# PaddlePaddle/PaddleRec

Hardware: AMD Instinct MI355X
Metric: CTR samples/sec, Criteo DeepFM bs=65536 (train step: fwd+bwd+optimizer) (higher is better)
Workload: dtype f32 (MLP GEMMs: f32 operands as 3 bf16 terms, 6 bf16 MFMAs per product, f32 accumulate); 1 GPU; DeepFM full Criteo: 26 sparse slots x 1000000 rows x dim 16, 13 dense, MLP 400,400,400, batch 65536 per GPU, lazy Adam, uniform ids; global_batch=65536, parallelism=single, table_rows_total=26000000, index_oob_flag=0

## Files before the change

### paddlerec_amd/csrc/crossnet_layers.hip

```cpp
#include "rec_common.h"

namespace rec {

__global__ __launch_bounds__(kBlock) void add_into_kernel(int64_t n, float* __restrict__ dst,
                                                          const float* __restrict__ src, int accumulate) {
  for (int64_t i = (int64_t)blockIdx.x * kBlock + threadIdx.x; i < n; i += (int64_t)gridDim.x * kBlock)
    dst[i] = accumulate ? dst[i] + src[i] : src[i];
}

static void add_into(int64_t n, float* dst, const float* src, int accumulate, hipStream_t st) {
  int64_t grid = (n + kBlock - 1) / kBlock;
  if (grid > kNumCU * 8) grid = kNumCU * 8;
  hipLaunchKernelGGL(add_into_kernel, dim3((unsigned)grid), dim3(kBlock), 0, st, n, dst, src, accumulate);
}

struct Carve {
  char* base;
  size_t off = 0;
  explicit Carve(void* p) : base((char*)p) {}
  float* take(size_t floats) {
    float* r = base ? (float*)(base + off) : nullptr;
    off += align_up(floats * sizeof(float), 256);
    return r;
  }
};

static rec_gemm_desc gd(int64_t m, int n, int k, int lda, int ldb, int ldc, int ta, int tb, int epi) {
  rec_gemm_desc d;
  d.m = m; d.n = n; d.k = k; d.lda = lda; d.ldb = ldb; d.ldc = ldc;
  d.trans_a = ta; d.trans_b = tb; d.epilogue = epi; d.split_k = 0;
  return d;
}

static size_t gemm_ws(const rec_gemm_desc& d) {
  size_t b = 0;
  rec_gemm_f32_workspace_bytes(&d, &b);
  return align_up(b, 256);
}

static size_t max2(size_t a, size_t b) { return a > b ? a : b; }

}

using namespace rec;

#define REC_TRY(call)        \
  do {                       \
    if (int rc_ = (call)) return rc_; \
  } while (0)

static int v2_check(const rec_crossnet_v2_desc* d) {
  REC_REQUIRE(d, REC_EINVAL, "desc is NULL");
  REC_REQUIRE(d->batch >= 0 && d->d > 0, REC_EINVAL, "bad sizes B=%lld d=%d", (long long)d->batch, d->d);
  return REC_OK;
}
static int ldx(int ld, int d) { return ld > 0 ? ld : d; }
static int v2_ldmax(const rec_crossnet_v2_desc* d) {
  int m = d->d;
  for (int v : {d->ld_x0, d->ld_xl, d->ld_out, d->ld_u}) m = v > m ? v : m;
  return m;
}
static int mix_ldmax(const rec_crossnet_mix_desc* d) {
  int m = d->d;
  for (int v : {d->ld_x0, d->ld_xl, d->ld_out}) m = v > m ? v : m;
  return m;
}

extern "C" int rec_crossnet_v2_layer_workspace_bytes(const rec_crossnet_v2_desc* d, size_t* fwd_bytes,
                                                     size_t* bwd_bytes) {
  REC_TRY(v2_check(d));
  const int n = d->d;
  const int lw = v2_ldmax(d);
  if (fwd_bytes) *fwd_bytes = gemm_ws(gd(d->batch, n, n, lw, n, lw, 0, 0, REC_EPI_CROSS));
  if (bwd_bytes) {
    const size_t g = max2(gemm_ws(gd(n, n, (int)d->batch, lw, n, n, 1, 0, REC_EPI_NONE)),
                          gemm_ws(gd(d->batch, n, n, n, n, lw, 0, 1, REC_EPI_ADD)));
    *bwd_bytes = align_up((size_t)d->batch * n * sizeof(float), 256) + g;
  }
  return REC_OK;
}

extern "C" int rec_crossnet_v2_layer_fwd(const rec_crossnet_v2_desc* d, const float* X0, const float* Xl,
                                         const float* W, const float* bias, float* Xnext, float* U_saved,
                                         void* workspace, size_t workspace_bytes, void* stream) {
  REC_TRY(v2_check(d));
  if (d->batch == 0) return REC_OK;
  REC_REQUIRE(X0 && Xl && W && bias && Xnext, REC_EINVAL, "null pointer argument");
  const int n = d->d;
  const rec_gemm_desc g = gd(d->batch, n, n, ldx(d->ld_xl, n), n, ldx(d->ld_out, n), 0, 0, REC_EPI_CROSS);
  rec_gemm_epilogue_args a = {};
  a.bias = bias;
  a.aux0 = X0; a.ld_aux0 = ldx(d->ld_x0, n);
  a.aux1 = Xl; a.ld_aux1 = ldx(d->ld_xl, n);
  a.out2 = U_saved; a.ld_out2 = ldx(d->ld_u, n);
  return rec_gemm_f32(&g, Xl, W, Xnext, &a, workspace, workspace_bytes, stream);
}

extern "C" int rec_crossnet_v2_layer_bwd(const rec_crossnet_v2_desc* d, const float* X0, const float* Xl,
                                         const float* W, const float* U_saved, const float* dXnext,
                                         int32_t ld_dxnext, float* dX0_acc, int32_t ld_acc,
                                         int32_t accumulate_dx0, int32_t fold_dx0, float* dXl, int32_t ld_dxl,
                                         float* dW, float* db, void* workspace, size_t workspace_bytes,
                                         void* stream) {
  REC_TRY(v2_check(d));
  if (d->batch == 0) return REC_OK;
  REC_REQUIRE(X0 && Xl && W && U_saved && dXnext && dX0_acc && dXl && dW && db, REC_EINVAL,
              "null pointer argument");
  const int n = d->d;
  size_t need = 0;
  rec_crossnet_v2_layer_workspace_bytes(d, nullptr, &need);
  REC_REQUIRE(workspace && workspace_bytes >= need, REC_EWORKSPACE, "workspace %zu < %zu", workspace_bytes, need);
  Carve c(workspace);
  float* dU = c.take((size_t)d->batch * n);
  void* gws = (char*)workspace + c.off;
  const size_t gws_bytes = workspace_bytes - c.off;
  REC_TRY(rec_cross_bwd_prep(d->batch, n, dXnext, ldx(ld_dxnext, n), X0, ldx(d->ld_x0, n), U_saved,
                             ldx(d->ld_u, n), dU, n, dX0_acc, ldx(ld_acc, n), accumulate_dx0, stream));
  {
    const rec_gemm_desc g = gd(n, n, (int)d->batch, ldx(d->ld_xl, n), n, n, 1, 0, REC_EPI_NONE);
    rec_gemm_epilogue_args a = {};
    a.b_colsum = db;
    REC_TRY(rec_gemm_f32(&g, Xl, dU, dW, &a, gws, gws_bytes, stream));
  }
  {
    const rec_gemm_desc g = gd(d->batch, n, n, n, n, ldx(ld_dxl, n), 0, 1, REC_EPI_ADD);
    rec_gemm_epilogue_args a = {};
    a.aux1 = dXnext; a.ld_aux1 = ldx(ld_dxnext, n);
    if (fold_dx0) { a.aux0 = dX0_acc; a.ld_aux0 = ldx(ld_acc, n); }
    REC_TRY(rec_gemm_f32(&g, dU, W, dXl, &a, gws, gws_bytes, stream));
  }
  return REC_OK;
}

static int mix_check(const rec_crossnet_mix_desc* d) {
  REC_REQUIRE(d, REC_EINVAL, "desc is NULL");
  REC_REQUIRE(d->batch >= 0 && d->d > 0 && d->rank > 0 && d->experts > 0 && d->experts <= 64, REC_EINVAL,
              "bad sizes B=%lld d=%d r=%d E=%d", (long long)d->batch, d->d, d->rank, d->experts);
  return REC_OK;
}

static size_t mix_gemm_ws(const rec_crossnet_mix_desc* d) {
  const int n = d->d, r = d->rank, E = d->experts;
  const int64_t B = d->batch;
  const int lw = mix_ldmax(d);
  size_t g = 0;
  g = max2(g, gemm_ws(gd(B, E, n, lw, E, E, 0, 0, REC_EPI_BIAS)));
  g = max2(g, gemm_ws(gd(B, r, n, lw, r, E * r, 0, 0, REC_EPI_BIAS_TANH)));
  g = max2(g, gemm_ws(gd(B, r, r, E * r, r, E * r, 0, 1, REC_EPI_BIAS_TANH)));
  g = max2(g, gemm_ws(gd(B, n, r, E * r, r, lw, 0, 1, REC_EPI_MOE)));
  g = max2(g, gemm_ws(gd(n, r, (int)B, lw, E * r, r, 1, 0, REC_EPI_NONE)));
  g = max2(g, gemm_ws(gd(r, r, (int)B, r, E * r, r, 1, 0, REC_EPI_NONE)));
  g = max2(g, gemm_ws(gd(B, r, n, n, r, r, 0, 0, REC_EPI_DTANH)));
  g = max2(g, gemm_ws(gd(B, r, r, r, r, r, 0, 0, REC_EPI_DTANH)));
  g = max2(g, gemm_ws(gd(B, n, r, r, r, lw, 0, 1, REC_EPI_ADD)));
  g = max2(g, gemm_ws(gd(n, E, (int)B, lw, E, E, 1, 0, REC_EPI_NONE)));
  g = max2(g, gemm_ws(gd(B, n, E, E, E, lw, 0, 1, REC_EPI_ADD)));
  size_t cs = 0;
  rec_colsum_workspace_bytes(B, n, &cs);
  return max2(g, align_up(cs, 256));
}

extern "C" int rec_crossnet_mix_layer_workspace_bytes(const rec_crossnet_mix_desc* d, size_t* fwd_bytes,
                                                      size_t* bwd_bytes) {
  REC_TRY(mix_check(d));
  const size_t B = (size_t)d->batch, n = d->d, r = d->rank, E = d->experts;
  const size_t g = mix_gemm_ws(d);
  auto al = [](size_t floats) { return align_up(floats * sizeof(float), 256); };
  if (fwd_bytes) *fwd_bytes = al(B * E) + g;
  if (bwd_bytes)
    *bwd_bytes = 2 * al(B * n) + al(B * E) + 2 * al(B * r) + al(B * E) + al(n) + al(n * E) + al(E) + g;
  return REC_OK;
}

extern "C" int rec_crossnet_mix_layer_fwd(const rec_crossnet_mix_desc* d, const float* X0, const float* Xl,
                                          const float* U, const float* V, const float* Cm, const float* bias,
                                          const float* gate_w, const float* gate_b, float* Xnext, float* t1,
                                          float* t2, float* prob, void* workspace, size_t workspace_bytes,
                                          void* stream) {
  REC_TRY(mix_check(d));
  if (d->batch == 0) return REC_OK;
  REC_REQUIRE(X0 && Xl && U && V && Cm && bias && gate_w && gate_b && Xnext && t1 && t2 && prob, REC_EINVAL,
              "null pointer argument");
  const int n = d->d, r = d->rank, E = d->experts;
  const int64_t B = d->batch;
  const int lx0 = ldx(d->ld_x0, n), lxl = ldx(d->ld_xl, n), lo = ldx(d->ld_out, n);
  size_t need = 0;
  rec_crossnet_mix_layer_workspace_bytes(d, &need, nullptr);
  REC_REQUIRE(workspace && workspace_bytes >= need, REC_EWORKSPACE, "workspace %zu < %zu", workspace_bytes, need);
  Carve c(workspace);
  float* gate = c.take((size_t)B * E);
  void* gws = (char*)workspace + c.off;
  const size_t gwb = workspace_bytes - c.off;
  {
    const rec_gemm_desc g = gd(B, E, n, lxl, E, E, 0, 0, REC_EPI_BIAS);
    rec_gemm_epilogue_args a = {};
    a.bias = gate_b;
    REC_TRY(rec_gemm_f32(&g, Xl, gate_w, gate, &a, gws, gwb, stream));
  }
  REC_TRY(rec_softmax_rows(B, E, gate, E, prob, E, stream));
  for (int e = 0; e < E; ++e) {
    {
      const rec_gemm_desc g = gd(B, r, n, lxl, r, E * r, 0, 0, REC_EPI_BIAS_TANH);
      rec_gemm_epilogue_args a = {};
      REC_TRY(rec_gemm_f32(&g, Xl, V + (size_t)e * n * r, t1 + e * r, &a, gws, gwb, stream));
    }
    {
      const rec_gemm_desc g = gd(B, r, r, E * r, r, E * r, 0, 1, REC_EPI_BIAS_TANH);
      rec_gemm_epilogue_args a = {};
      REC_TRY(rec_gemm_f32(&g, t1 + e * r, Cm + (size_t)e * r * r, t2 + e * r, &a, gws, gwb, stream));
    }
  }
  for (int e = 0; e < E; ++e) {
    const rec_gemm_desc g = gd(B, n, r, E * r, r, lo, 0, 1, REC_EPI_MOE);
    rec_gemm_epilogue_args a = {};
    a.bias = bias;
    a.aux0 = X0; a.ld_aux0 = lx0;
    a.aux1 = e == 0 ? Xl : Xnext; a.ld_aux1 = e == 0 ? lxl : lo;
    a.row_scale = prob + e; a.row_scale_stride = E;
    REC_TRY(rec_gemm_f32(&g, t2 + e * r, U + (size_t)e * n * r, Xnext, &a, gws, gwb, stream));
  }
  return REC_OK;
}

extern "C" int rec_crossnet_mix_layer_bwd(const rec_crossnet_mix_desc* d, const float* X0, const float* Xl,
                                          const float* U, const float* V, const float* Cm, const float* bias,
                                          const float* gate_w, const float* t1, const float* t2,
                                          const float* prob, const float* dXnext, int32_t ld_dxnext,
                                          float* dX0_acc, int32_t ld_acc, int32_t accumulate_dx0,
                                          int32_t fold_dx0, float* dXl, int32_t ld_dxl, float* gU, float* gV,
                                          float* gC, float* gbias, float* g_gate_w, float* g_gate_b,
                                          int32_t accumulate_gate, void* workspace, size_t workspace_bytes,
                                          void* stream) {
  REC_TRY(mix_check(d));
  if (d->batch == 0) return REC_OK;
  REC_REQUIRE(X0 && Xl && U && V && Cm && bias && gate_w && t1 && t2 && prob && dXnext && dX0_acc && dXl && gU &&
                  gV && gC && gbias && g_gate_w && g_gate_b, REC_EINVAL, "null pointer argument");
  REC_REQUIRE(dXl != dXnext, REC_EINVAL, "dXl must not alias dXnext (every expert reads dXnext)");
  const int n = d->d, r = d->rank, E = d->experts;
  const int64_t B = d->batch;
  const int lx0 = ldx(d->ld_x0, n), lxl = ldx(d->ld_xl, n), ldn = ldx(ld_dxnext, n), lacc = ldx(ld_acc, n),
            ldl = ldx(ld_dxl, n);
  hipStream_t st = (hipStream_t)stream;
  size_t need = 0;
  rec_crossnet_mix_layer_workspace_bytes(d, nullptr, &need);
  REC_REQUIRE(workspace && workspace_bytes >= need, REC_EWORKSPACE, "workspace %zu < %zu", workspace_bytes, need);
  Carve c(workspace);
  float* u = c.take((size_t)B * n);
  float* du = c.take((size_t)B * n);
  float* dp = c.take((size_t)B * E);
  float* dc = c.take((size_t)B * r);
  float* da = c.take((size_t)B * r);
  float* dgate = c.take((size_t)B * E);
  float* dbias_e = c.take(n);
  float* gw = c.take((size_t)n * E);
  float* gb = c.take(E);
  void* gws = (char*)workspace + c.off;
  const size_t gwb = workspace_bytes - c.off;
  int acc = accumulate_dx0;
  for (int e = 0; e < E; ++e) {
    const float* t1e = t1 + e * r;
    const float* t2e = t2 + e * r;
    const float* Ue = U + (size_t)e * n * r;
    const float* Ve = V + (size_t)e * n * r;
    const float* Ce = Cm + (size_t)e * r * r;
    rec_gemm_epilogue_args a;
    {
      const rec_gemm_desc g = gd(B, n, r, E * r, r, n, 0, 1, REC_EPI_BIAS);
      a = {}; a.bias = bias;
      REC_TRY(rec_gemm_f32(&g, t2e, Ue, u, &a, gws, gwb, stream));
    }
    REC_TRY(rec_moe_bwd_prep(B, n, dXnext, ldn, X0, lx0, u, n, prob + e, E, du, n, dX0_acc, lacc, acc, dp + e, E,
                             stream));
    acc = 1;
    REC_TRY(rec_colsum(B, n, n, du, dbias_e, gws, gwb, stream));
    add_into(n, gbias, dbias_e, e > 0, st);
    {
      const rec_gemm_desc g = gd(n, r, (int)B, n, E * r, r, 1, 0, REC_EPI_NONE);
      a = {};
      REC_TRY(rec_gemm_f32(&g, du, t2e, gU + (size_t)e * n * r, &a, gws, gwb, stream));
    }
    {
      const rec_gemm_desc g = gd(B, r, n, n, r, r, 0, 0, REC_EPI_DTANH);
      a = {}; a.aux0 = t2e; a.ld_aux0 = E * r;
      REC_TRY(rec_gemm_f32(&g, du, Ue, dc, &a, gws, gwb, stream));
    }
    {
      const rec_gemm_desc g = gd(r, r, (int)B, r, E * r, r, 1, 0, REC_EPI_NONE);
      a = {};
      REC_TRY(rec_gemm_f32(&g, dc, t1e, gC + (size_t)e * r * r, &a, gws, gwb, stream));
    }
    {
      const rec_gemm_desc g = gd(B, r, r, r, r, r, 0, 0, REC_EPI_DTANH);
      a = {}; a.aux0 = t1e; a.ld_aux0 = E * r;
      REC_TRY(rec_gemm_f32(&g, dc, Ce, da, &a, gws, gwb, stream));
    }
    {
      const rec_gemm_desc g = gd(n, r, (int)B, lxl, r, r, 1, 0, REC_EPI_NONE);
      a = {};
      REC_TRY(rec_gemm_f32(&g, Xl, da, gV + (size_t)e * n * r, &a, gws, gwb, stream));
    }
    {
      const rec_gemm_desc g = gd(B, n, r, r, r, ldl, 0, 1, REC_EPI_ADD);
      a = {};
      a.aux1 = e == 0 ? dXnext : dXl; a.ld_aux1 = e == 0 ? ldn : ldl;
      REC_TRY(rec_gemm_f32(&g, da, Ve, dXl, &a, gws, gwb, stream));
    }
  }
  REC_TRY(rec_softmax_rows_bwd(B, E, prob, E, dp, E, dgate, E, stream));
  {
    rec_gemm_epilogue_args a = {};
    const rec_gemm_desc g1 = gd(n, E, (int)B, lxl, E, E, 1, 0, REC_EPI_NONE);
    REC_TRY(rec_gemm_f32(&g1, Xl, dgate, gw, &a, gws, gwb, stream));
    add_into((int64_t)n * E, g_gate_w, gw, accumulate_gate, st);
    REC_TRY(rec_colsum(B, E, E, dgate, gb, gws, gwb, stream));
    add_into(E, g_gate_b, gb, accumulate_gate, st);
    const rec_gemm_desc g2 = gd(B, n, E, E, E, ldl, 0, 1, REC_EPI_ADD);
    a = {};
    a.aux1 = dXl; a.ld_aux1 = ldl;
    if (fold_dx0) { a.aux0 = dX0_acc; a.ld_aux0 = lacc; }
    REC_TRY(rec_gemm_f32(&g2, dgate, gate_w, dXl, &a, gws, gwb, stream));
  }
  return check_launch("rec_crossnet_mix_layer_bwd");
}
```

### paddlerec_amd/csrc/gemm_bf16x3.h

```cpp
#pragma once

#include <atomic>

#include "gemm_epi.h"
#include "gemm_glds.h"

namespace rec {

typedef __bf16 bf16x8_t __attribute__((ext_vector_type(8)));
typedef unsigned u32x4_t __attribute__((ext_vector_type(4)));

constexpr int kX3NT = 13;
constexpr int kX3NP = 2 * kX3NT * 16;
constexpr int kX3BM = 128;
constexpr int kX3MT = 4;
constexpr int kX3Stage = 3 * kX3NP * 64;
template <int NT>
struct X3Geo {
  static constexpr int NP = NT * 16;
  static constexpr int Plane = NP * 64;
  static constexpr int Stage = 3 * Plane;
  static constexpr int Pieces = Stage / 1024;
};
struct X3Cols { int nt, ncb; };
// ... 338 lines not shown
          if (epi.out2) *reinterpret_cast<f32x4_t*>(epi.out2 + i * epi.ld2 + j) = u;
        }
      }
    }
    if constexpr (EPI == REC_EPI_BIAS_RELU) {
      if (bits_at && row_ok) *bits_at = mbits;
    }
  }
}

constexpr int kX3DwCols = 208;
constexpr int kX3DwPlane = kX3DwCols * 64;
constexpr int kX3DwOperand = 3 * kX3DwPlane;
constexpr int kX3DwWT = 7;

__device__ __forceinline__ int x3_dw_q(int i, int a) { return (i >> 2) + 4 * (((i & 3) + a) & 3); }

template <int T>
__device__ __forceinline__ void x3_dw_read(u32x4_t (&f)[3], unsigned base) {
  asm volatile("ds_read_b128 %0, %1 offset:%2" : "=v"(f[0]) : "v"(base), "n"(T * 256));
  asm volatile("ds_read_b128 %0, %1 offset:%2" : "=v"(f[1]) : "v"(base), "n"(T * 256 + kX3DwPlane));
  asm volatile("ds_read_b128 %0, %1 offset:%2" : "=v"(f[2]) : "v"(base), "n"(T * 256 + 2 * kX3DwPlane));
}

__device__ __forceinline__ void x3_dw_read_u(u32x4_t (&f)[3], unsigned base, int u) {
  switch (u) {
    case 0: x3_dw_read<0>(f, base); break;
    case 1: x3_dw_read<1>(f, base); break;
    case 2: x3_dw_read<2>(f, base); break;
    case 3: x3_dw_read<3>(f, base); break;
    case 4: x3_dw_read<4>(f, base); break;
    case 5: x3_dw_read<5>(f, base); break;
    default: x3_dw_read<6>(f, base); break;
  }
}

__device__ __forceinline__ void x3_dw_wait_frags(u32x4_t (&f)[3], int left) {
#define REC_X3_WAIT_CASE(N) case N: asm volatile("s_waitcnt lgkmcnt(" #N ")" : "+v"(f[0]), "+v"(f[1]), "+v"(f[2])); break;
  switch (left) {
    REC_X3_WAIT_CASE(0) REC_X3_WAIT_CASE(1) REC_X3_WAIT_CASE(2) REC_X3_WAIT_CASE(3) REC_X3_WAIT_CASE(4) REC_X3_WAIT_CASE(5)
    REC_X3_WAIT_CASE(6) REC_X3_WAIT_CASE(7) REC_X3_WAIT_CASE(8) REC_X3_WAIT_CASE(9) REC_X3_WAIT_CASE(10) REC_X3_WAIT_CASE(11)
    REC_X3_WAIT_CASE(12) REC_X3_WAIT_CASE(13) REC_X3_WAIT_CASE(14) REC_X3_WAIT_CASE(15)
    default: asm volatile("s_waitcnt lgkmcnt(0)" : "+v"(f[0]), "+v"(f[1]), "+v"(f[2])); break;
  }
#undef REC_X3_WAIT_CASE
}

struct X3DwArgs {
  const float* X; int64_t ldx;
  const float* G; int64_t ldg;
  int64_t rows;
  int kin, nout;
  int kb_tiles, nb_tiles;
  int kblocks, nblocks;
  int slices, steps_per_slice;
  float* P; int64_t ldp;
  float* cpart;
};

template <int PW, bool PIPE>
__global__ __launch_bounds__(256) void gemm_bf16x3_dw_kernel(X3DwArgs w) {
  extern __shared__ __attribute__((aligned(1024))) char x3_smem[];
  const int tid = threadIdx.x;
  const int lane = tid % kWave;
  const int wave = __builtin_amdgcn_readfirstlane(tid / kWave);
  const int li = lane & 15, g = lane >> 4;
  const int wk = wave & 1, wn = wave >> 1;
  const int nob = w.kblocks * w.nblocks;
  const int xcd = blockIdx.x & 7, j = blockIdx.x >> 3;
  const int ob = j % nob, slice = (j / nob) * 8 + xcd;
  const int kb = ob / w.nblocks, nb = ob % w.nblocks;
  const int k_tile0 = kb * w.kb_tiles, n_tile0 = nb * w.nb_tiles;
  const int kt_blk = min(w.kb_tiles, (w.kin + 15) / 16 - k_tile0);
  const int nt_blk = min(w.nb_tiles, (w.nout + 15) / 16 - n_tile0);
  const int k_split = (kt_blk + 1) / 2, n_split = (nt_blk + 1) / 2;
  const int my_k0 = wk ? k_split : 0, my_p = __builtin_amdgcn_readfirstlane(wk ? kt_blk - k_split : k_split);
  const int my_n0 = wn ? n_split : 0, my_q = __builtin_amdgcn_readfirstlane(wn ? nt_blk - n_split : n_split);
  const int64_t row0 = (int64_t)slice * w.steps_per_slice * 32;
  int nsteps = (int)min((int64_t)w.steps_per_slice, (w.rows - row0) / 32);
  if (nsteps < 0) nsteps = 0;

  const bool stager = tid < 4 * (kX3DwCols / 4);
  const int mg = stager ? tid / (kX3DwCols / 4) : 0, cg = tid % (kX3DwCols / 4);
  const int xc = k_tile0 * 16 + cg * 4, gc = n_tile0 * 16 + cg * 4;
  const bool x_ok = stager && cg * 4 < kt_blk * 16 && xc < w.kin;
  const bool g_ok = stager && cg * 4 < nt_blk * 16 && gc < w.nout;
  const float* xp = w.X + (row0 + mg * 8) * w.ldx + (x_ok ? xc : 0);
  const float* gp = w.G + (row0 + mg * 8) * w.ldg + (g_ok ? gc : 0);
  float4 xr[8], gr[8];
  auto load_patches = [&](int kt) {
#ifdef REC_X3_DW_NO_LOADS
    if (kt > 0) return;
#endif
#pragma unroll
    for (int r = 0; r < 8; ++r) {
      xr[r] = *reinterpret_cast<const float4*>(xp + ((int64_t)kt * 32 + r) * w.ldx);
      gr[r] = *reinterpret_cast<const float4*>(gp + ((int64_t)kt * 32 + r) * w.ldg);
    }
  };
  unsigned wr_off[4];
#pragma unroll
  for (int e = 0; e < 4; ++e) {
    const int a = cg >> 2, i = 4 * (cg & 3) + e;
    wr_off[e] = (unsigned)((mg * kX3DwCols + 16 * a + x3_dw_q(i, a)) * 16);
  }
  float4 csum = make_float4(0.f, 0.f, 0.f, 0.f);
  const unsigned w_stage = stager ? (unsigned)kX3Stage : 0u, w_oper = stager ? (unsigned)kX3DwOperand : 0u,
                 w_plane = stager ? (unsigned)kX3DwPlane : 0u;
  char* const w_base = stager ? x3_smem : x3_smem + 2 * kX3Stage + tid * 16;
  if (!stager) { wr_off[0] = wr_off[1] = wr_off[2] = wr_off[3] = 0u; }
  auto convert_compute = [&](int e, u32x4_t (&ch)[6]) {
    float xv[8], gv[8];
#pragma unroll
    for (int r = 0; r < 8; ++r) {
      xv[r] = e == 0 ? xr[r].x : e == 1 ? xr[r].y : e == 2 ? xr[r].z : xr[r].w;
      gv[r] = e == 0 ? gr[r].x : e == 1 ? gr[r].y : e == 2 ? gr[r].z : gr[r].w;
    }
    asm volatile("" : "+v"(xv[0]), "+v"(xv[1]), "+v"(xv[2]), "+v"(xv[3]), "+v"(xv[4]), "+v"(xv[5]), "+v"(xv[6]), "+v"(xv[7]),
                      "+v"(gv[0]), "+v"(gv[1]), "+v"(gv[2]), "+v"(gv[3]), "+v"(gv[4]), "+v"(gv[5]), "+v"(gv[6]), "+v"(gv[7]));
#pragma unroll
    for (int d = 0; d < 4; ++d) {
      unsigned a, b, c;
#ifdef REC_X3_DW_NOCVT
      a = __float_as_uint(xv[2 * d]); b = __float_as_uint(xv[2 * d + 1]); c = a ^ b;
#else
      x3_split_pair(x_ok ? xv[2 * d] : 0.f, x_ok ? xv[2 * d + 1] : 0.f, a, b, c);
#endif
      ch[0][d] = a; ch[1][d] = b; ch[2][d] = c;
    }
    float cs = 0.f;
#pragma unroll
    for (int d = 0; d < 4; ++d) {
      const float u0 = g_ok ? gv[2 * d] : 0.f, u1 = g_ok ? gv[2 * d + 1] : 0.f;
      cs += u0 + u1;
      unsigned a, b, c;
#ifdef REC_X3_DW_NOCVT
      a = __float_as_uint(u0); b = __float_as_uint(u1); c = a ^ b;
#else
      x3_split_pair(u0, u1, a, b, c);
#endif
      ch[3][d] = a; ch[4][d] = b; ch[5][d] = c;
    }
    if (e == 0) csum.x += cs; else if (e == 1) csum.y += cs; else if (e == 2) csum.z += cs; else csum.w += cs;
  };
  auto convert_write = [&](int stage, int e, const u32x4_t (&ch)[6]) {
    char* sx = w_base + stage * w_stage + wr_off[e];
    char* sg = sx + w_oper;
#ifdef REC_X3_DW_NOWRITE
    *reinterpret_cast<u32x4_t*>(sx) = ch[0] ^ ch[1] ^ ch[2];
    *reinterpret_cast<u32x4_t*>(sg) = ch[3] ^ ch[4] ^ ch[5];
#else
    *reinterpret_cast<u32x4_t*>(sx) = ch[0];
    *reinterpret_cast<u32x4_t*>(sx + w_plane) = ch[1];
    *reinterpret_cast<u32x4_t*>(sx + 2 * w_plane) = ch[2];
    *reinterpret_cast<u32x4_t*>(sg) = ch[3];
    *reinterpret_cast<u32x4_t*>(sg + w_plane) = ch[4];
    *reinterpret_cast<u32x4_t*>(sg + 2 * w_plane) = ch[5];
#endif
  };
  auto convert_part = [&](int stage, int e) {
    u32x4_t ch[6];
    convert_compute(e, ch);
    convert_write(stage, e, ch);
  };
  auto convert_store = [&](int stage) {
#pragma unroll
    for (int e = 0; e < 4; ++e) convert_part(stage, e);
  };

  f32x4_t acc[PW][kX3DwWT];
#pragma unroll
  for (int a = 0; a < PW; ++a)
#pragma unroll
    for (int t = 0; t < kX3DwWT; ++t) acc[a][t] = f32x4_t{0.f, 0.f, 0.f, 0.f};

  const unsigned lds0 = (unsigned)(uintptr_t)x3_smem;
  unsigned xb[4], gb[4];
#pragma unroll
  for (int u = 0; u < 4; ++u) {
    const int ax = my_k0 + u, an = my_n0 + u;
    xb[u] = lds0 + (unsigned)((g * kX3DwCols + 16 * my_k0 + x3_dw_q(li, ax)) * 16);
    gb[u] = lds0 + kX3DwOperand + (unsigned)((g * kX3DwCols + 16 * my_n0 + x3_dw_q(li, an)) * 16);
  }

  if (nsteps > 0) {
    load_patches(0);
    convert_store(0);
  }
  __syncthreads();

  auto step = [&](int kt, auto more_c) {
    constexpr bool MORE = decltype(more_c)::value;
    const int stage = kt & 1;
    if (MORE) load_patches(kt + 1);
    __builtin_amdgcn_sched_barrier(0);
    const unsigned so = stage * kX3Stage;
    u32x4_t af[PW][3];
    u32x4_t bf[2][3];
    u32x4_t pend[6];
    x3_dw_read_u(bf[0], gb[0] + so, 0);
#pragma unroll
    for (int u = 0; u < PW; ++u) x3_dw_read_u(af[u], xb[u & 3] + so, u);
    x3_dw_read_u(bf[1], gb[1] + so, 1);
#pragma unroll
    for (int a = 0; a < PW; ++a) {
      x3_dw_wait_frags(af[a], 3 * (PW - 1 - a) + 3);
      const u32x4_t* b0 = bf[0];
#define REC_X3_DW_MFMA0(PB, PA)                                                                                \
  acc[a][0] = __builtin_amdgcn_mfma_f32_16x16x32_bf16(__builtin_bit_cast(bf16x8_t, b0[PB]),                      \
                                                      __builtin_bit_cast(bf16x8_t, af[a][PA]), acc[a][0], 0, 0, 0);
#if REC_X3_PRODUCTS >= 6
      REC_X3_DW_MFMA0(2, 0) REC_X3_DW_MFMA0(1, 1) REC_X3_DW_MFMA0(0, 2)
#endif
#if REC_X3_PRODUCTS >= 3
      REC_X3_DW_MFMA0(1, 0) REC_X3_DW_MFMA0(0, 1)
#endif
      REC_X3_DW_MFMA0(0, 0)
#undef REC_X3_DW_MFMA0
      __builtin_amdgcn_sched_barrier(0);
    }
    __builtin_amdgcn_sched_barrier(0);
#pragma unroll
    for (int t = 1; t < kX3DwWT; ++t) {
      if (t + 1 < kX3DwWT) {
        x3_dw_read_u(bf[(t + 1) & 1], gb[(t + 1) & 3] + so, t + 1);
        asm volatile("s_waitcnt lgkmcnt(3)" : "+v"(bf[t & 1][0]), "+v"(bf[t & 1][1]), "+v"(bf[t & 1][2]));
      } else {
        asm volatile("s_waitcnt lgkmcnt(0)" : "+v"(bf[t & 1][0]), "+v"(bf[t & 1][1]), "+v"(bf[t & 1][2]));
      }
      const u32x4_t* b = bf[t & 1];
#define REC_X3_DW_MFMA(PB, PA)                                                                                 \
  _Pragma("unroll") for (int a = 0; a < PW; ++a) acc[a][t] = __builtin_amdgcn_mfma_f32_16x16x32_bf16(            \
      __builtin_bit_cast(bf16x8_t, b[PB]), __builtin_bit_cast(bf16x8_t, af[a][PA]), acc[a][t], 0, 0, 0);
#if REC_X3_PRODUCTS >= 6
      REC_X3_DW_MFMA(2, 0) REC_X3_DW_MFMA(1, 1) REC_X3_DW_MFMA(0, 2)
#endif
#if REC_X3_PRODUCTS >= 3
      REC_X3_DW_MFMA(1, 0) REC_X3_DW_MFMA(0, 1)
#endif
      REC_X3_DW_MFMA(0, 0)
#undef REC_X3_DW_MFMA
#ifndef REC_X3_DW_SERIAL_CONVERT
      if constexpr (PIPE) {
      if (MORE && t >= kX3DwWT - 5) {
        const bool wr = t >= kX3DwWT - 4, cv = t <= kX3DwWT - 2;
        if (wr) convert_write(stage ^ 1, t - (kX3DwWT - 4), pend);
        if (cv) convert_compute(t - (kX3DwWT - 5), pend);
#pragma unroll
        for (int i = 0; i < 6 * PW; ++i) {
          __builtin_amdgcn_sched_group_barrier(0x008, 1, 0);
          if (cv) __builtin_amdgcn_sched_group_barrier(0x002, REC_X3_DW_VALU_PER_MFMA, 0);
          if (wr && i % PW == PW / 2) __builtin_amdgcn_sched_group_barrier(0x200, 1, 0);
        }
        if (cv) __builtin_amdgcn_sched_group_barrier(0x002, 32, 0);
      }
      } else if (MORE && t >= kX3DwWT - 4) {
        convert_part(stage ^ 1, t - (kX3DwWT - 4));
#pragma unroll
        for (int i = 0; i < 6 * PW; ++i) {
          __builtin_amdgcn_sched_group_barrier(0x008, 1, 0);
          __builtin_amdgcn_sched_group_barrier(0x002, REC_X3_DW_VALU_PER_MFMA, 0);
        }
        __builtin_amdgcn_sched_group_barrier(0x002, 32, 0);
        __builtin_amdgcn_sched_group_barrier(0x200, 6, 0);
      }
#endif
      __builtin_amdgcn_sched_barrier(0);
    }
#ifdef REC_X3_DW_SERIAL_CONVERT
    if (MORE) convert_store(stage ^ 1);
#endif
    __syncthreads();
  };
  for (int kt = 0; kt + 1 < nsteps; ++kt) step(kt, std::true_type{});
  if (nsteps > 0) step(nsteps - 1, std::false_type{});

  float* P = w.P + (int64_t)slice * w.kin * w.ldp;
#pragma unroll
  for (int a = 0; a < PW; ++a) {
    if (a >= my_p) continue;
    const int ki = (k_tile0 + my_k0 + a) * 16 + li;
#pragma unroll
    for (int t = 0; t < kX3DwWT; ++t) {
      if (t >= my_q) continue;
      const int nj = (n_tile0 + my_n0 + t) * 16 + g * 4;
      if (ki < w.kin && nj < w.nout) *reinterpret_cast<f32x4_t*>(P + (int64_t)ki * w.ldp + nj) = acc[a][t];
    }
  }
  if (w.cpart && kb == 0) {
    float4* red = reinterpret_cast<float4*>(x3_smem);
    if (stager) red[(tid / (kX3DwCols / 4)) * (kX3DwCols / 4) + cg] = csum;
    __syncthreads();
    if (tid < kX3DwCols / 4 && tid * 4 < nt_blk * 16 && n_tile0 * 16 + tid * 4 < w.nout) {
      const float4 s0 = red[tid], s1 = red[kX3DwCols / 4 + tid], s2 = red[2 * (kX3DwCols / 4) + tid],
                   s3 = red[3 * (kX3DwCols / 4) + tid];
      float4 o;
      o.x = (s0.x + s1.x) + (s2.x + s3.x); o.y = (s0.y + s1.y) + (s2.y + s3.y);
      o.z = (s0.z + s1.z) + (s2.z + s3.z); o.w = (s0.w + s1.w) + (s2.w + s3.w);
      *reinterpret_cast<float4*>(w.cpart + (int64_t)slice * w.nout + n_tile0 * 16 + tid * 4) = o;
    }
  }
}

inline int x3_launch_split(const float* W, int64_t ldw, int K, int N, int trans, char* img, hipStream_t st) {
  const X3Cols c = x3_cols(N);
  const int nkt = (K + 31) / 32, np = c.nt * 16, ncb = 2 * c.ncb;
  const int64_t thr = (int64_t)ncb * nkt * np * 4;
  hipLaunchKernelGGL(x3_split_kernel, dim3((unsigned)((thr + kBlock - 1) / kBlock)), dim3(kBlock), 0, st, W, ldw, K, N,
                     trans, img, nkt, np, ncb);
  return check_launch("x3_split_kernel");
}

inline size_t x3_relu_bits_bytes(int64_t M, int N) { return (size_t)M * (2 * x3_cols(N).ncb) * 4 * sizeof(unsigned long long); }

inline bool x3_shape_ok(int64_t M, int N, int K, int64_t lda, int64_t ldc, const void* A, const void* C) {
  return M > 0 && N > 0 && x3_cols(N).nt > 0 && N % 4 == 0 && K > 0 && K % 8 == 0 && lda % 4 == 0 && ldc % 4 == 0 &&
         ((uintptr_t)A % 16) == 0 && ((uintptr_t)C % 16) == 0;
}

template <int NT, int EPI, int WM, int WN>
inline int x3_launch_gemm_wm(int64_t M, int N, int K, const float* A, int64_t lda, const char* img, float* C, int64_t ldc,
                             const EpiArgs& e, int ncb, hipStream_t st) {
  static std::atomic<bool> attr_set{false};
  constexpr int lds = 2 * WN * X3Geo<NT>::Stage;
  if (!attr_set.load(std::memory_order_acquire)) {
    if (hipFuncSetAttribute(reinterpret_cast<const void*>(&gemm_bf16x3_kernel<NT, EPI, WM, WN>),
                            hipFuncAttributeMaxDynamicSharedMemorySize, lds) != hipSuccess) {
      (void)hipGetLastError();
      set_error("gemm_bf16x3: %d B of dynamic LDS refused", lds);
      return REC_EHIP;
    }
    attr_set.store(true, std::memory_order_release);
  }
  const int64_t row_tiles = (M + kX3BM - 1) / kX3BM;
  if constexpr (WN == 1) {
    const int64_t grid = (row_tiles + 7) / 8 * 8 * ncb;
    if (grid >= (1ll << 31)) { set_error("gemm_bf16x3: too many workgroups"); return REC_ESHAPE; }
    hipLaunchKernelGGL((gemm_bf16x3_kernel<NT, EPI, WM, WN>), dim3((unsigned)grid), dim3(WM * WN * 64), lds, st, M, N, K, A,
                       lda, img, C, ldc, e, ncb);
  } else {
    hipLaunchKernelGGL((gemm_bf16x3_kernel<NT, EPI, WM, WN>), dim3((unsigned)row_tiles, (unsigned)(ncb / WN)),
                       dim3(WM * WN * 64), lds, st, M, N, K, A, lda, img, C, ldc, e, ncb);
  }
  return check_launch("gemm_bf16x3_kernel");
}

#ifndef REC_X3_WM
#define REC_X3_WM 4
#endif
inline int x3_wn_default() {
  static const int v = [] { const char* e = getenv("REC_X3_WN"); return e && *e == '2' ? 2 : 1; }();
  return v;
}
template <int NT, int EPI>
inline int x3_launch_gemm_cfg(int64_t M, int N, int K, const float* A, int64_t lda, const char* img, float* C, int64_t ldc,
                              const EpiArgs& e, int ncb, hipStream_t st) {
  if constexpr (EpiUses<EPI>::aux1) {
    return x3_launch_gemm_wm<NT, EPI, 2, 2>(M, N, K, A, lda, img, C, ldc, e, ncb, st);
  } else {
    if (REC_X3_WM == 4 && x3_wn_default() == 1)
      return x3_launch_gemm_wm<NT, EPI, 4, 1>(M, N, K, A, lda, img, C, ldc, e, ncb, st);
    return x3_launch_gemm_wm<NT, EPI, REC_X3_WM, 2>(M, N, K, A, lda, img, C, ldc, e, ncb, st);
  }
}

template <int EPI>
inline int x3_launch_gemm_epi(int64_t M, int N, int K, const float* A, int64_t lda, const char* img, float* C, int64_t ldc,
                              const EpiArgs& e, hipStream_t st) {
  const X3Cols c = x3_cols(N);
  switch (c.nt) {
    case 13: return x3_launch_gemm_cfg<13, EPI>(M, N, K, A, lda, img, C, ldc, e, 2 * c.ncb, st);
    case 8: return x3_launch_gemm_cfg<8, EPI>(M, N, K, A, lda, img, C, ldc, e, 2 * c.ncb, st);
    case 7: return x3_launch_gemm_cfg<7, EPI>(M, N, K, A, lda, img, C, ldc, e, 2 * c.ncb, st);
    default: set_error("gemm_bf16x3: no column blocking for N = %d", N); return REC_ESHAPE;
  }
}

inline bool x3_epilogue_ok(int epi) { return epi >= REC_EPI_NONE && epi <= REC_EPI_DTANH; }

inline int x3_launch_gemm(int epi, int64_t M, int N, int K, const float* A, int64_t lda, const char* img, float* C,
                          int64_t ldc, const EpiArgs& e, hipStream_t st) {
  switch (epi) {
    case REC_EPI_NONE: return x3_launch_gemm_epi<REC_EPI_NONE>(M, N, K, A, lda, img, C, ldc, e, st);
    case REC_EPI_BIAS: return x3_launch_gemm_epi<REC_EPI_BIAS>(M, N, K, A, lda, img, C, ldc, e, st);
    case REC_EPI_BIAS_RELU: return x3_launch_gemm_epi<REC_EPI_BIAS_RELU>(M, N, K, A, lda, img, C, ldc, e, st);
    case REC_EPI_RELU_MASK: return x3_launch_gemm_epi<REC_EPI_RELU_MASK>(M, N, K, A, lda, img, C, ldc, e, st);
    case REC_EPI_CROSS: return x3_launch_gemm_epi<REC_EPI_CROSS>(M, N, K, A, lda, img, C, ldc, e, st);
    case REC_EPI_BIAS_SIGMOID: return x3_launch_gemm_epi<REC_EPI_BIAS_SIGMOID>(M, N, K, A, lda, img, C, ldc, e, st);
    case REC_EPI_BIAS_TANH: return x3_launch_gemm_epi<REC_EPI_BIAS_TANH>(M, N, K, A, lda, img, C, ldc, e, st);
    case REC_EPI_ADD: return x3_launch_gemm_epi<REC_EPI_ADD>(M, N, K, A, lda, img, C, ldc, e, st);
    case REC_EPI_MOE: return x3_launch_gemm_epi<REC_EPI_MOE>(M, N, K, A, lda, img, C, ldc, e, st);
    case REC_EPI_DSIGMOID: return x3_launch_gemm_epi<REC_EPI_DSIGMOID>(M, N, K, A, lda, img, C, ldc, e, st);
    case REC_EPI_DTANH: return x3_launch_gemm_epi<REC_EPI_DTANH>(M, N, K, A, lda, img, C, ldc, e, st);
    default: set_error("gemm_bf16x3: epilogue %d not built", epi); return REC_EINVAL;
  }
}

struct X3DwPlan { int kb_tiles, nb_tiles, kblocks, nblocks, slices, steps_per_slice; };
inline bool x3_dw_plan(int kin, int nout, int64_t rows, int cus, X3DwPlan* p) {
  if (kin % 4 || nout % 4 || rows % 32 || kin < 16 || nout < 16) return false;
  const int kt = (kin + 15) / 16, nt = (nout + 15) / 16;
  p->kblocks = (kt + 12) / 13; p->nblocks = (nt + 12) / 13;
  p->kb_tiles = (kt + p->kblocks - 1) / p->kblocks; p->nb_tiles = (nt + p->nblocks - 1) / p->nblocks;
  const int nob = p->kblocks * p->nblocks;
  int slices = cus / nob;
  slices -= slices % 8;
  if (slices < 8) return false;
  const int64_t steps = rows / 32;
  p->steps_per_slice = (int)((steps + slices - 1) / slices);
  if (p->steps_per_slice < 4) return false;
  p->slices = (int)((steps + p->steps_per_slice - 1) / p->steps_per_slice);
  p->slices = (p->slices + 7) / 8 * 8;
  return true;
}
inline int x3_launch_dw(const X3DwPlan& pl, int kin, int nout, int64_t rows, const float* X, int64_t ldx, const float* G,
                        int64_t ldg, float* P, int64_t ldp, float* cpart, hipStream_t st) {
  static std::atomic<bool> attr_set{false};
  constexpr int lds = 2 * kX3Stage + 4096;
  if (!attr_set.load(std::memory_order_acquire)) {
    if (hipFuncSetAttribute(reinterpret_cast<const void*>(&gemm_bf16x3_dw_kernel<7, true>),
                            hipFuncAttributeMaxDynamicSharedMemorySize, lds) != hipSuccess ||
        hipFuncSetAttribute(reinterpret_cast<const void*>(&gemm_bf16x3_dw_kernel<5, true>),
                            hipFuncAttributeMaxDynamicSharedMemorySize, lds) != hipSuccess ||
        hipFuncSetAttribute(reinterpret_cast<const void*>(&gemm_bf16x3_dw_kernel<7, false>),
                            hipFuncAttributeMaxDynamicSharedMemorySize, lds) != hipSuccess ||
        hipFuncSetAttribute(reinterpret_cast<const void*>(&gemm_bf16x3_dw_kernel<5, false>),
                            hipFuncAttributeMaxDynamicSharedMemorySize, lds) != hipSuccess) {
      (void)hipGetLastError();
      set_error("gemm_bf16x3_dw: %d B of dynamic LDS refused", lds);
      return REC_EHIP;
    }
    attr_set.store(true, std::memory_order_release);
  }
  X3DwArgs w{X, ldx, G, ldg, rows, kin, nout, pl.kb_tiles, pl.nb_tiles, pl.kblocks, pl.nblocks, pl.slices,
             pl.steps_per_slice, P, ldp, cpart};
  const unsigned grid = (unsigned)(pl.slices * pl.kblocks * pl.nblocks);
  static const bool pipe = [] { const char* v = getenv("REC_X3_DW_PIPE"); return v && *v ? *v != '0' : REC_X3_DW_PIPE_STORES != 0; }();
  const bool p5 = (pl.kb_tiles + 1) / 2 <= 5;
  if (p5 && pipe) hipLaunchKernelGGL((gemm_bf16x3_dw_kernel<5, true>), dim3(grid), dim3(256), lds, st, w);
  else if (p5) hipLaunchKernelGGL((gemm_bf16x3_dw_kernel<5, false>), dim3(grid), dim3(256), lds, st, w);
  else if (pipe) hipLaunchKernelGGL((gemm_bf16x3_dw_kernel<7, true>), dim3(grid), dim3(256), lds, st, w);
  else hipLaunchKernelGGL((gemm_bf16x3_dw_kernel<7, false>), dim3(grid), dim3(256), lds, st, w);
  return check_launch("gemm_bf16x3_dw_kernel");
}

}
```

Measured before the change: 42.48 million samples/s.

## Add 8-wave weight-gradient bf16x3 GEMM kernel and make it default

Adds a new 512-thread weight-gradient kernel in which eight waves split the K tiles four ways and the N tiles two ways, with half the threads staging X and half staging G. It interleaves global loads, bf16 splitting and LDS writes with the MFMA stream using sched_group_barrier hints. The kernel is on by default through a compile-time flag and an env var. The aim is more waves per block to hide latency and fewer accumulator registers per wave, at the cost of extra synchronisation and register pressure.

```diff
diff --git a/paddlerec_amd/csrc/crossnet_layers.hip b/paddlerec_amd/csrc/crossnet_layers.hip
--- a/paddlerec_amd/csrc/crossnet_layers.hip
+++ b/paddlerec_amd/csrc/crossnet_layers.hip
@@ -26,7 +26,7 @@
 };
 
 static rec_gemm_desc gd(int64_t m, int n, int k, int lda, int ldb, int ldc, int ta, int tb, int epi) {
-  rec_gemm_desc d;
+  rec_gemm_desc d{};
   d.m = m; d.n = n; d.k = k; d.lda = lda; d.ldb = ldb; d.ldc = ldc;
   d.trans_a = ta; d.trans_b = tb; d.epilogue = epi; d.split_k = 0;
   return d;
diff --git a/paddlerec_amd/csrc/gemm_bf16x3.h b/paddlerec_amd/csrc/gemm_bf16x3.h
--- a/paddlerec_amd/csrc/gemm_bf16x3.h
+++ b/paddlerec_amd/csrc/gemm_bf16x3.h
@@ -664,6 +664,217 @@
   }
 }
 
+template <int PW>
+struct X3Dw8Acc { f32x4_t v[PW][kX3DwWT]; };
+
+struct X3Dw8Ctx {
+  const float* src; int64_t ld; bool ok;
+  char* base; unsigned wr_off[4];
+  unsigned xb[4], gb[4];
+  float4 raw[8];
+  float4 csum;
+  float* P; int64_t ldp; int kin, nout, k_tile0, n_tile0, my_k0, my_n0, my_p, my_q, li, g;
+  __device__ __forceinline__ void load_patch(int kt) {
+#pragma unroll
+    for (int r = 0; r < 8; ++r) raw[r] = *reinterpret_cast<const float4*>(src + ((int64_t)kt * 32 + r) * ld);
+  }
+  __device__ __forceinline__ void convert(int e, u32x4_t (&ch)[3]) {
+    float v[8];
+#pragma unroll
+    for (int r = 0; r < 8; ++r) v[r] = e == 0 ? raw[r].x : e == 1 ? raw[r].y : e == 2 ? raw[r].z : raw[r].w;
+    asm volatile("" : "+v"(v[0]), "+v"(v[1]), "+v"(v[2]), "+v"(v[3]), "+v"(v[4]), "+v"(v[5]), "+v"(v[6]), "+v"(v[7]));
+    float cs = 0.f;
+#pragma unroll
+    for (int d = 0; d < 4; ++d) {
+      const float u0 = ok ? v[2 * d] : 0.f, u1 = ok ? v[2 * d + 1] : 0.f;
+      cs += u0 + u1;
+      unsigned a, b, cc;
+      x3_split_pair(u0, u1, a, b, cc);
+      ch[0][d] = a; ch[1][d] = b; ch[2][d] = cc;
+    }
+    if (e == 0) csum.x += cs; else if (e == 1) csum.y += cs; else if (e == 2) csum.z += cs; else csum.w += cs;
+  }
+  __device__ __forceinline__ void write(int stage, int e, const u32x4_t (&ch)[3]) {
+    char* p = base + stage * kX3Stage + wr_off[e];
+    *reinterpret_cast<u32x4_t*>(p) = ch[0];
+    *reinterpret_cast<u32x4_t*>(p + kX3DwPlane) = ch[1];
+    *reinterpret_cast<u32x4_t*>(p + 2 * kX3DwPlane) = ch[2];
+  }
+  template <int NP>
+  __device__ __forceinline__ void store(const f32x4_t (&acc)[NP][kX3DwWT]) {
+#pragma unroll
+    for (int a = 0; a < NP; ++a) {
+      if (a >= my_p) continue;
+      const int ki = (k_tile0 + my_k0 + a) * 16 + li;
+#pragma unroll
+      for (int t = 0; t < kX3DwWT; ++t) {
+        if (t >= my_q) continue;
+        const int nj = (n_tile0 + my_n0 + t) * 16 + g * 4;
+        if (ki < kin && nj < nout) *reinterpret_cast<f32x4_t*>(P + (int64_t)ki * ldp + nj) = acc[a][t];
+      }
+    }
+  }
+};
+
+template <int PW>
+__device__ __forceinline__ void x3_dw8_run(X3Dw8Ctx& c, int nsteps) {
+  X3Dw8Acc<PW> acc;
+#pragma unroll
+  for (int a = 0; a < PW; ++a)
+#pragma unroll
+    for (int t = 0; t < kX3DwWT; ++t) acc.v[a][t] = f32x4_t{0.f, 0.f, 0.f, 0.f};
+  auto step = [&](int kt, auto more_c) {
+    constexpr bool MORE = decltype(more_c)::value;
+    const int stage = kt & 1;
+    if (MORE) c.load_patch(kt + 1);
+    __builtin_amdgcn_sched_barrier(0);
+    const unsigned so = stage * kX3Stage;
+    u32x4_t af[PW][3];
+    u32x4_t bf[2][3];
+    u32x4_t pend[3];
+    x3_dw_read_u(bf[0], c.gb[0] + so, 0);
+#pragma unroll
+    for (int u = 0; u < PW; ++u) x3_dw_read_u(af[u], c.xb[u & 3] + so, u);
+    x3_dw_read_u(bf[1], c.gb[1] + so, 1);
+#pragma unroll
+    for (int a = 0; a < PW; ++a) {
+      x3_dw_wait_frags(af[a], 3 * (PW - 1 - a) + 3);
+      const u32x4_t* b0 = bf[0];
+#define REC_X3_DW8_MFMA0(PB, PA)                                                                               \
+  acc.v[a][0] = __builtin_amdgcn_mfma_f32_16x16x32_bf16(__builtin_bit_cast(bf16x8_t, b0[PB]),                  \
+                                                        __builtin_bit_cast(bf16x8_t, af[a][PA]), acc.v[a][0], 0, 0, 0);
+#if REC_X3_PRODUCTS >= 6
+      REC_X3_DW8_MFMA0(2, 0) REC_X3_DW8_MFMA0(1, 1) REC_X3_DW8_MFMA0(0, 2)
+#endif
+#if REC_X3_PRODUCTS >= 3
+      REC_X3_DW8_MFMA0(1, 0) REC_X3_DW8_MFMA0(0, 1)
+#endif
+      REC_X3_DW8_MFMA0(0, 0)
+#undef REC_X3_DW8_MFMA0
+      __builtin_amdgcn_sched_barrier(0);
+    }
+    __builtin_amdgcn_sched_barrier(0);
+#pragma unroll
+    for (int t = 1; t < kX3DwWT; ++t) {
+      if (t + 1 < kX3DwWT) {
+        x3_dw_read_u(bf[(t + 1) & 1], c.gb[(t + 1) & 3] + so, t + 1);
+        asm volatile("s_waitcnt lgkmcnt(3)" : "+v"(bf[t & 1][0]), "+v"(bf[t & 1][1]), "+v"(bf[t & 1][2]));
+      } else {
+        asm volatile("s_waitcnt lgkmcnt(0)" : "+v"(bf[t & 1][0]), "+v"(bf[t & 1][1]), "+v"(bf[t & 1][2]));
+      }
+      const u32x4_t* b = bf[t & 1];
+#define REC_X3_DW8_MFMA(PB, PA)                                                                                \
+  _Pragma("unroll") for (int a = 0; a < PW; ++a) acc.v[a][t] = __builtin_amdgcn_mfma_f32_16x16x32_bf16(        \
+      __builtin_bit_cast(bf16x8_t, b[PB]), __builtin_bit_cast(bf16x8_t, af[a][PA]), acc.v[a][t], 0, 0, 0);
+#if REC_X3_PRODUCTS >= 6
+      REC_X3_DW8_MFMA(2, 0) REC_X3_DW8_MFMA(1, 1) REC_X3_DW8_MFMA(0, 2)
+#endif
+#if REC_X3_PRODUCTS >= 3
+      REC_X3_DW8_MFMA(1, 0) REC_X3_DW8_MFMA(0, 1)
+#endif
+      REC_X3_DW8_MFMA(0, 0)
+#undef REC_X3_DW8_MFMA
+      if (MORE && t >= kX3DwWT - 5) {
+        const bool wr = t >= kX3DwWT - 4, cv = t <= kX3DwWT - 2;
+        if (wr) c.write(stage ^ 1, t - (kX3DwWT - 4), pend);
+        if (cv) c.convert(t - (kX3DwWT - 5), pend);
+#pragma unroll
+        for (int i = 0; i < 6 * PW; ++i) {
+          __builtin_amdgcn_sched_group_barrier(0x008, 1, 0);
+          if (cv) __builtin_amdgcn_sched_group_barrier(0x002, REC_X3_DW_VALU_PER_MFMA, 0);
+          if (wr && i % (2 * PW) == PW) __builtin_amdgcn_sched_group_barrier(0x200, 1, 0);
+        }
+        if (cv) __builtin_amdgcn_sched_group_barrier(0x002, 32, 0);
+      }
+      __builtin_amdgcn_sched_barrier(0);
+    }
+    __syncthreads();
+  };
+  for (int kt = 0; kt + 1 < nsteps; ++kt) step(kt, std::true_type{});
+  if (nsteps > 0) step(nsteps - 1, std::false_type{});
+  c.store(acc.v);
+}
+
+template <int PW>
+__global__ __launch_bounds__(512) void gemm_bf16x3_dw_kernel_w8(X3DwArgs w) {
+  static_assert(PW >= 2 && PW <= 4, "four X tiles at most fit the 256-register budget");
+  extern __shared__ __attribute__((aligned(1024))) char x3_smem[];
+  const int tid = threadIdx.x;
+  const int lane = tid % kWave;
+  const int wave = __builtin_amdgcn_readfirstlane(tid / kWave);
+  const int li = lane & 15, g = lane >> 4;
+  const int wk = wave < 4 ? wave : 7 - wave, wn = wave >> 2;
+  const int nob = w.kblocks * w.nblocks;
+  const int xcd = blockIdx.x & 7, j = blockIdx.x >> 3;
+  const int ob = j % nob, slice = (j / nob) * 8 + xcd;
+  const int kb = ob / w.nblocks, nb = ob % w.nblocks;
+  const int k_tile0 = kb * w.kb_tiles, n_tile0 = nb * w.nb_tiles;
+  const int kt_blk = min(w.kb_tiles, (w.kin + 15) / 16 - k_tile0);
+  const int nt_blk = min(w.nb_tiles, (w.nout + 15) / 16 - n_tile0);
+  const int n_split = (nt_blk + 1) / 2;
+  const int kq = kt_blk >> 2, kr = kt_blk & 3;
+  const int my_k0 = wk * kq + min(wk, kr), my_p = __builtin_amdgcn_readfirstlane(kq + (wk < kr ? 1 : 0));
+  const int my_n0 = wn ? n_split : 0, my_q = __builtin_amdgcn_readfirstlane(wn ? nt_blk - n_split : n_split);
+  const int64_t row0 = (int64_t)slice * w.steps_per_slice * 32;
+  int nsteps = (int)min((int64_t)w.steps_per_slice, (w.rows - row0) / 32);
+  if (nsteps < 0) nsteps = 0;
+
+  const int op = wave >> 2, s = tid & 255;
+  const bool stager = s < 4 * (kX3DwCols / 4);
+  const int sp = stager ? s : s - 4 * (kX3DwCols / 4);
+  const int mg = sp / (kX3DwCols / 4), cg = sp % (kX3DwCols / 4);
+  const int col = (op ? n_tile0 : k_tile0) * 16 + cg * 4;
+  const bool ok = cg * 4 < (op ? nt_blk : kt_blk) * 16 && col < (op ? w.nout : w.kin);
+  const int64_t ld = op ? w.ldg : w.ldx;
+  const float* src = (op ? w.G : w.X) + (row0 + mg * 8) * ld + (ok ? col : 0);
+
+  X3Dw8Ctx c;
+  c.src = src; c.ld = ld; c.ok = ok;
+  c.base = x3_smem + op * kX3DwOperand;
+#pragma unroll
+  for (int e = 0; e < 4; ++e) {
+    const int a = cg >> 2, i = 4 * (cg & 3) + e;
+    c.wr_off[e] = (unsigned)((mg * kX3DwCols + 16 * a + x3_dw_q(i, a)) * 16);
+  }
+  c.csum = make_float4(0.f, 0.f, 0.f, 0.f);
+  const unsigned lds0 = (unsigned)(uintptr_t)x3_smem;
+#pragma unroll
+  for (int u = 0; u < 4; ++u) {
+    const int ax = my_k0 + u, an = my_n0 + u;
+    c.xb[u] = lds0 + (unsigned)((g * kX3DwCols + 16 * my_k0 + x3_dw_q(li, ax)) * 16);
+    c.gb[u] = lds0 + kX3DwOperand + (unsigned)((g * kX3DwCols + 16 * my_n0 + x3_dw_q(li, an)) * 16);
+  }
+  c.P = w.P + (int64_t)slice * w.kin * w.ldp; c.ldp = w.ldp; c.kin = w.kin; c.nout = w.nout; c.k_tile0 = k_tile0; c.n_tile0 = n_tile0; c.my_k0 = my_k0; c.my_n0 = my_n0;
+  c.my_p = my_p; c.my_q = my_q; c.li = li; c.g = g;
+
+  if (nsteps > 0) {
+    c.load_patch(0);
+#pragma unroll
+    for (int e = 0; e < 4; ++e) {
+      u32x4_t ch[3];
+      c.convert(e, ch);
+      c.write(0, e, ch);
+    }
+  }
+  __syncthreads();
+  if (my_p == PW) x3_dw8_run<PW>(c, nsteps);
+  else x3_dw8_run<PW - 1>(c, nsteps);
+
+  if (w.cpart && kb == 0) {
+    float4* red = reinterpret_cast<float4*>(x3_smem);
+    if (op == 1 && stager) red[mg * (kX3DwCols / 4) + cg] = c.csum;
+    __syncthreads();
+    if (tid < kX3DwCols / 4 && tid * 4 < nt_blk * 16 && n_tile0 * 16 + tid * 4 < w.nout) {
+      const float4 s0 = red[tid], s1 = red[kX3DwCols / 4 + tid], s2 = red[2 * (kX3DwCols / 4) + tid],
+                   s3 = red[3 * (kX3DwCols / 4) + tid];
+      float4 o;
+      o.x = (s0.x + s1.x) + (s2.x + s3.x); o.y = (s0.y + s1.y) + (s2.y + s3.y);
+      o.z = (s0.z + s1.z) + (s2.z + s3.z); o.w = (s0.w + s1.w) + (s2.w + s3.w);
+      *reinterpret_cast<float4*>(w.cpart + (int64_t)slice * w.nout + n_tile0 * 16 + tid * 4) = o;
+    }
+  }
+}
+
 inline int x3_launch_split(const float* W, int64_t ldw, int K, int N, int trans, char* img, hipStream_t st) {
   const X3Cols c = x3_cols(N);
   const int nkt = (K + 31) / 32, np = c.nt * 16, ncb = 2 * c.ncb;
@@ -775,19 +986,21 @@
   p->slices = (p->slices + 7) / 8 * 8;
   return true;
 }
+#ifndef REC_X3_DW_FORM_DEFAULT
+#define REC_X3_DW_FORM_DEFAULT 1
+#endif
+template <typename K>
+inline bool x3_dw_lds_attr(K kernel, int lds) {
+  return hipFuncSetAttribute(reinterpret_cast<const void*>(kernel), hipFuncAttributeMaxDynamicSharedMemorySize, lds) == hipSuccess;
+}
 inline int x3_launch_dw(const X3DwPlan& pl, int kin, int nout, int64_t rows, const float* X, int64_t ldx, const float* G,
-                        int64_t ldg, float* P, int64_t ldp, float* cpart, hipStream_t st) {
+                        int64_t ldg, float* P, int64_t ldp, float* cpart, hipStream_t st, int form = -1) {
   static std::atomic<bool> attr_set{false};
   constexpr int lds = 2 * kX3Stage + 4096;
   if (!attr_set.load(std::memory_order_acquire)) {
-    if (hipFuncSetAttribute(reinterpret_cast<const void*>(&gemm_bf16x3_dw_kernel<7, true>),
-                            hipFuncAttributeMaxDynamicSharedMemorySize, lds) != hipSuccess ||
-        hipFuncSetAttribute(reinterpret_cast<const void*>(&gemm_bf16x3_dw_kernel<5, true>),
-                            hipFuncAttributeMaxDynamicSharedMemorySize, lds) != hipSuccess ||
-        hipFuncSetAttribute(reinterpret_cast<const void*>(&gemm_bf16x3_dw_kernel<7, false>),
-                            hipFuncAttributeMaxDynamicSharedMemorySize, lds) != hipSuccess ||
-        hipFuncSetAttribute(reinterpret_cast<const void*>(&gemm_bf16x3_dw_kernel<5, false>),
-                            hipFuncAttributeMaxDynamicSharedMemorySize, lds) != hipSuccess) {
+    if (!x3_dw_lds_attr(&gemm_bf16x3_dw_kernel<7, true>, lds) || !x3_dw_lds_attr(&gemm_bf16x3_dw_kernel<5, true>, lds) ||
+        !x3_dw_lds_attr(&gemm_bf16x3_dw_kernel<7, false>, lds) || !x3_dw_lds_attr(&gemm_bf16x3_dw_kernel<5, false>, lds) ||
+        !x3_dw_lds_attr(&gemm_bf16x3_dw_kernel_w8<4>, lds) || !x3_dw_lds_attr(&gemm_bf16x3_dw_kernel_w8<3>, lds)) {
       (void)hipGetLastError();
       set_error("gemm_bf16x3_dw: %d B of dynamic LDS refused", lds);
       return REC_EHIP;
@@ -797,6 +1010,15 @@
   X3DwArgs w{X, ldx, G, ldg, rows, kin, nout, pl.kb_tiles, pl.nb_tiles, pl.kblocks, pl.nblocks, pl.slices,
              pl.steps_per_slice, P, ldp, cpart};
   const unsigned grid = (unsigned)(pl.slices * pl.kblocks * pl.nblocks);
+  static const int env_form = [] {
+    const char* v = getenv("REC_X3_DW_FORM");
+    return v && *v ? (*v != '0' ? 1 : 0) : REC_X3_DW_FORM_DEFAULT;
+  }();
+  if ((form < 0 ? env_form : form) != 0) {
+    if ((pl.kb_tiles + 3) / 4 >= 4) hipLaunchKernelGGL((gemm_bf16x3_dw_kernel_w8<4>), dim3(grid), dim3(512), lds, st, w);
+    else hipLaunchKernelGGL((gemm_bf16x3_dw_kernel_w8<3>), dim3(grid), dim3(512), lds, st, w);
+    return check_launch("gemm_bf16x3_dw_kernel_w8");
+  }
   static const bool pipe = [] { const char* v = getenv("REC_X3_DW_PIPE"); return v && *v ? *v != '0' : REC_X3_DW_PIPE_STORES != 0; }();
   const bool p5 = (pl.kb_tiles + 1) / 2 <= 5;
   if (p5 && pipe) hipLaunchKernelGGL((gemm_bf16x3_dw_kernel<5, true>), dim3(grid), dim3(256), lds, st, w);
```

Result: faster. 43.53 million samples/s, median of 6 (+2.5%).
